# Farama-Foundation/Miniworld

Hardware: NVIDIA H100
Metric: env steps/sec (higher is better)
Workload: dtype f64+f32

## Files before the change

### miniworld_b200/csrc/mwb.cu

```cuda
#include <math.h>
#include <stdio.h>
#include <stdlib.h>
#include <string.h>

#include <algorithm>
#include <string>
#include <vector>

#include "../../include/mwb.h"
#include "raster.cuh"
#include "visibility.cuh"
#include "reset.cuh"

#ifndef MWB_HOSTSIM
#include <cuda_runtime.h>
#endif

#define MWB_MAX_ENTS_CAP 32
#define MWB_STAGE_QUAD_BYTES_HOST 16384

static thread_local std::string g_err;
static int fail(int code, const std::string& msg) {
  g_err = msg;
  return code;
}

#ifdef MWB_HOSTSIM
typedef void* stream_t;
static int dev_alloc(void** p, size_t n) {
  *p = calloc(1, n ? n : 1);
  return *p ? 0 : -1;
}
static void dev_free(void* p) { free(p); }
static int h2d(void* d, const void* h, size_t n, stream_t) { memcpy(d, h, n); return 0; }
static int d2h(void* h, const void* d, size_t n, stream_t) { memcpy(h, d, n); return 0; }
static int dev_memset(void* d, int v, size_t n) { memset(d, v, n); return 0; }
static int sync_stream(stream_t) { return 0; }
static bool is_device_ptr(const void*) { return false; }
#else
typedef cudaStream_t stream_t;
#define CK(call)                                                                              \
  do {                                                                                        \
    cudaError_t e_ = (call);                                                                  \
    if (e_ != cudaSuccess)                                                                    \
      return fail(MWB_ECUDA, std::string(#call) + " (mwb.cu:" + std::to_string(__LINE__) + "): " + cudaGetErrorString(e_)); \
  } while (0)
static int dev_alloc(void** p, size_t n) { return cudaMalloc(p, n ? n : 1) == cudaSuccess ? 0 : -1; }
static void dev_free(void* p) { cudaFree(p); }
static int h2d(void* d, const void* h, size_t n, stream_t s) {
  return cudaMemcpyAsync(d, h, n, cudaMemcpyHostToDevice, s) == cudaSuccess ? 0 : -1;
}
static int d2h(void* h, const void* d, size_t n, stream_t s) {
  return cudaMemcpyAsync(h, d, n, cudaMemcpyDeviceToHost, s) == cudaSuccess ? 0 : -1;
}
static int dev_memset(void* d, int v, size_t n) {
  return cudaMemset(d, v, n) == cudaSuccess && cudaStreamSynchronize(cudaStreamLegacy) == cudaSuccess ? 0 : -1;
}
static int sync_stream(stream_t s) { return cudaStreamSynchronize(s) == cudaSuccess ? 0 : -1; }
static bool is_device_ptr(const void* p) {
  if (!p) return false;
  cudaPointerAttributes a;
  if (cudaPointerGetAttributes(&a, p) != cudaSuccess) {
    cudaGetLastError();
    return false;
  }
  return a.type == cudaMemoryTypeDevice || a.type == cudaMemoryTypeManaged;
}
#endif

struct WorldUpload {
  int32_t env, num_slots, agent_slot, carrying, step_count, num_picked, hold, pad1;
  double cam[4];
  double envp[12];
  mwb_entity ents[MWB_MAX_ENTS_CAP];
  mwb_rng_state rng;
};

#define MWB_D2H_CHUNKS 16

struct mwb_handle {
  mwb_config cfg;
  DevState S;
  RenderAssets A;
  std::vector<void*> allocs;
  stream_t stream;
  int64_t launches;
  int32_t* d_actions;
  double* d_step_params;
  double* d_reward;
  uint8_t* d_term;
  uint8_t* d_trunc;
  uint8_t* d_obs;
  int obs_format;
  size_t obs_px_bytes;
  size_t d_obs_bytes;
  float* d_depth;
  int32_t* d_ids;
  int* d_overflow;
  WorldUpload* d_upload;
  int tri_cap;
  bool smem_tris;
  int stage_bytes;
  bool have_params, have_protos, have_template;
  bool have_level_table;
  std::vector<LevelDev> levels;
  std::vector<int32_t> env_level;
  std::vector<mwb_op> ops_h;
  int geom_blocks;
  bool profiling;
  bool frames_copied;
  int obs_peer_hint;
  const void* peer_checked;
  bool peer_result;
  bool obs_is_peer;
  int k2_static_smem;
  TriRec* vis_tris;
  ViewSpec view;
  int k2_parts;
#ifndef MWB_HOSTSIM
  cudaStream_t copy_stream;
  cudaEvent_t chunk_done[MWB_D2H_CHUNKS], copies_done;
#endif
#ifndef MWB_HOSTSIM
  std::vector<cudaEvent_t> ev_k1, ev_k2;
  cudaEvent_t last_done;
  cudaStream_t last_stream;
  bool last_valid;
#endif
#ifndef MWB_HOSTSIM
  struct AtlasEntry* atlas;
#endif
  std::vector<int> mesh_counts;
  void* mesh_tris_buf;
  void* mesh_bbox_buf;
  void* mesh_bin_idx_buf;
  void* mesh_bin_off_buf;
  void *tex_desc, *texels, *mesh_desc, *mesh_pos, *mesh_nrm, *mesh_uv, *mesh_rgb, *mesh_tex, *protos, *ops, *maze, *maze_cdf;
};

#ifndef MWB_HOSTSIM
struct AtlasEntry {
  int device;
  uint64_t hash;
  size_t texels;
  int refs;
  cudaArray_t arr;
  cudaTextureObject_t obj;
  float iw, ih;
  std::vector<float> ax, ay;
};
static std::vector<AtlasEntry*> g_atlases;
static void release_texture_objects(mwb_handle* h) {
  AtlasEntry* e = h->atlas;
  h->atlas = nullptr;
  if (!e || --e->refs > 0) return;
  for (size_t k = 0; k < g_atlases.size(); ++k)
    if (g_atlases[k] == e) g_atlases.erase(g_atlases.begin() + k);
  cudaDestroyTextureObject(e->obj);
  cudaFreeArray(e->arr);
  delete e;
}
#endif

template <typename T>
static int alloc_arr(mwb_handle* h, T** p, size_t count) {
  void* q = nullptr;
  if (dev_alloc(&q, count * sizeof(T)) != 0) return fail(MWB_ECUDA, "device allocation failed");
  dev_memset(q, 0, count * sizeof(T));
  h->allocs.push_back(q);
  *p = (T*)q;
  return 0;
}

#ifndef MWB_HOSTSIM
static int stream_enter(mwb_handle* h, stream_t s) {
  if (h->last_valid && h->last_stream != s) CK(cudaStreamWaitEvent(s, h->last_done, 0));
  return 0;
}
static int stream_leave(mwb_handle* h, stream_t s) {
  CK(cudaEventRecord(h->last_done, s));
  h->last_stream = s;
  h->last_valid = true;
  return 0;
}
#else
// ... 363 lines not shown
  h->tex_desc = h->texels = h->mesh_desc = h->mesh_pos = h->mesh_nrm = h->mesh_uv = h->mesh_rgb = h->mesh_tex = nullptr;
  h->protos = h->ops = h->maze = h->maze_cdf = nullptr;
  h->mesh_tris_buf = nullptr;
  h->mesh_bbox_buf = nullptr;
  h->mesh_bin_idx_buf = h->mesh_bin_off_buf = nullptr;
  memset(&h->view, 0, sizeof(ViewSpec));
  h->vis_tris = nullptr;
  h->obs_format = MWB_OBS_HWC_U8;
  h->obs_px_bytes = 3;
  h->obs_peer_hint = -1;
  h->peer_checked = nullptr;
  h->peer_result = h->obs_is_peer = false;
  h->k2_static_smem = 19456;
  memset(&h->S, 0, sizeof(DevState));
  memset(&h->A, 0, sizeof(RenderAssets));
#ifndef MWB_HOSTSIM
  if (cudaStreamCreateWithFlags(&h->stream, cudaStreamNonBlocking) != cudaSuccess ||
      cudaStreamCreateWithFlags(&h->copy_stream, cudaStreamNonBlocking) != cudaSuccess) {
    delete h;
    return fail(MWB_ECUDA, "cudaStreamCreate failed");
  }
  for (int c = 0; c < MWB_D2H_CHUNKS; ++c) cudaEventCreateWithFlags(&h->chunk_done[c], cudaEventDisableTiming);
  cudaEventCreateWithFlags(&h->copies_done, cudaEventDisableTiming);
  cudaEventCreateWithFlags(&h->last_done, cudaEventDisableTiming);
  h->last_stream = h->stream;
  h->last_valid = false;
#else
  h->stream = nullptr;
#endif
  DevState& S = h->S;
  const size_t N = cfg->num_envs, E = cfg->max_ents;
  S.N = cfg->num_envs;
  S.E = cfg->max_ents;
  S.R = cfg->max_rooms;
  S.Q = (cfg->max_quads + 1) & ~1;
  S.S = cfg->max_segs;
  S.shared_geom = cfg->shared_geometry;
  S.obs_w = cfg->obs_width;
  S.obs_h = cfg->obs_height;
  S.msaa = cfg->msaa_samples;
  S.domain_rand = cfg->domain_rand;
  S.autoreset = cfg->autoreset;
  {
    LevelDev L0;
    memset(&L0, 0, sizeof(L0));
    L0.rule_kind = cfg->rule_kind;
    L0.rule_arg = cfg->rule_arg;
    L0.max_episode_steps = cfg->max_episode_steps;
    h->levels.assign(1, L0);
    h->env_level.assign(N, 0);
    S.num_levels = 1;
  }
  const size_t G = cfg->shared_geometry ? 1 : N;
  h->geom_blocks = (int)G;
  int rc = 0;
#define AL(field, count) if (!rc) rc = alloc_arr(h, &S.field, (count))
  AL(ent_proto, E * N); AL(ent_px, E * N); AL(ent_py, E * N); AL(ent_pz, E * N); AL(ent_dir, E * N);
  AL(ent_col, E * 3 * N); AL(ent_size, E * N); AL(num_slots, N); AL(agent_slot, N); AL(carrying, N); AL(step_count, N);
  AL(num_picked, N); AL(needs_reset, N); AL(episodes_done, 1); AL(cam, 4 * N); AL(envp, 12 * N); AL(ghost_slot, N);
  AL(ghost_proto, N); AL(ghost_pose, 4 * N); AL(ghost_col, 3 * N);
  AL(rng_s_hi, N); AL(rng_s_lo, N); AL(rng_inc_hi, N); AL(rng_inc_lo, N); AL(rng_has32, N); AL(rng_cache, N);
  AL(num_rooms, G); AL(num_quads, G); AL(num_segs, G);
  AL(rooms, G * S.R); AL(quads, G * S.Q + 2); AL(segs, G * S.S); AL(room_tex, N * S.R * 3);
  AL(mesh_seg, N * E); AL(cam_trig, 6 * N); AL(ent_cs, E * 2 * N);
#undef AL
  LevelDev* d_levels = nullptr;
  int32_t* d_env_level = nullptr;
  if (!rc) rc = alloc_arr(h, &d_levels, MWB_LEVEL_CAP);
  if (!rc) rc = alloc_arr(h, &d_env_level, N);
  S.levels = d_levels;
  S.env_level = d_env_level;
  if (!rc) rc = alloc_arr(h, &h->d_actions, N);
  if (!rc) rc = alloc_arr(h, &h->d_step_params, 3 * N);
  if (!rc) rc = alloc_arr(h, &h->d_reward, N);
  if (!rc) rc = alloc_arr(h, &h->d_term, N);
  if (!rc) rc = alloc_arr(h, &h->d_trunc, N);
  if (!rc) rc = alloc_arr(h, &h->d_obs, N * (size_t)S.obs_w * S.obs_h * 3);
  h->d_obs_bytes = N * (size_t)S.obs_w * S.obs_h * 3;
  if (!rc) rc = alloc_arr(h, &h->d_depth, N * (size_t)S.obs_w * S.obs_h);
  if (!rc) rc = alloc_arr(h, &h->d_ids, N);
  if (!rc) rc = alloc_arr(h, &h->d_overflow, 1);
  S.fault = h->d_overflow;
  if (!rc) rc = alloc_arr(h, &h->d_upload, N);
  if (rc) {
    mwb_destroy(h);
    return rc;
  }
#ifndef MWB_HOSTSIM
  {
    float* lut = nullptr;
    if (alloc_arr(h, &lut, 65536)) {
      mwb_destroy(h);
      return fail(MWB_ECUDA, "depth table allocation failed");
    }
    depth_lut_kernel<<<256, 256, 0, h->stream>>>(lut);
    h->launches++;
    S.depth_lut = lut;
  }
#endif
  dev_memset(S.ent_proto, 0xFF, E * N * sizeof(int32_t));
  dev_memset(S.ghost_slot, 0xFF, N * sizeof(int32_t));
  dev_memset(S.carrying, 0xFF, N * sizeof(int32_t));
  {
    int sms = 132;
#ifndef MWB_HOSTSIM
    if (cudaDeviceGetAttribute(&sms, cudaDevAttrMultiProcessorCount, cfg->device) != cudaSuccess) {
      cudaGetLastError();
      sms = 132;
    }
#endif
    const int slots = 4 * 3 * sms;
    const int halves = ((cfg->obs_width + 7) / 8) * ((cfg->obs_height + 3) / 4);
    const int base = (halves + 149) / 150, want = (slots + cfg->num_envs - 1) / cfg->num_envs;
    const int maxp = halves / 30 > 1 ? halves / 30 : 1;
    h->k2_parts = base > want ? base : want;
    if (h->k2_parts > maxp) h->k2_parts = maxp;
    if (h->k2_parts < 1) h->k2_parts = 1;
  }
  h->tri_cap = 2 * (cfg->max_quads + 6 * cfg->max_ents) + 2;
  h->smem_tris = h->tri_cap <= 512;
  if (!h->smem_tris) {
    TriRec* buf = nullptr;
    if (alloc_arr(h, &buf, (size_t)N * h->k2_parts * h->tri_cap)) {
      mwb_destroy(h);
      return fail(MWB_ECUDA, "triangle list allocation failed");
    }
    S.room_tris = buf;
  }
  h->stage_bytes = (int)(((size_t)cfg->max_quads * sizeof(mwb_quad) + 15) & ~(size_t)15);
  if (h->stage_bytes > MWB_STAGE_QUAD_BYTES_HOST) h->stage_bytes = 0;
#ifndef MWB_HOSTSIM
  {
    cudaFuncAttributes fa;
    if (cudaFuncGetAttributes(&fa, k2_kernels[k2_index(h)]) == cudaSuccess) {
      h->k2_static_smem = (int)fa.sharedSizeBytes;
    } else {
      cudaGetLastError();
      h->k2_static_smem = 19456;
    }
  }
  const int smem = k2_smem_bytes(h) + 16384;
  if (ensure_k2_smem(h, smem)) {
    mwb_destroy(h);
    return fail(MWB_ECUDA, "cudaFuncSetAttribute(MaxDynamicSharedMemorySize) failed");
  }
  if (getenv("MWB_DEBUG")) {
    int nb = 0;
    const int launch_smem = k2_smem_bytes(h);
    cudaOccupancyMaxActiveBlocksPerMultiprocessor(&nb, k2_kernels[k2_index(h)], k2_threads(h), launch_smem);
    fprintf(stderr, "[mwb] K2 %d threads, %dx MSAA: dynamic smem %d B (local destination), parts %d, resident blocks/SM %d\n",
            k2_threads(h), h->S.msaa, launch_smem, h->k2_parts, nb);
  }
#endif
  *out = h;
  return MWB_OK;
}

extern "C" int mwb_destroy(mwb_handle* h) {
  if (!h) return MWB_OK;
#ifndef MWB_HOSTSIM
  cudaSetDevice(h->cfg.device);
  if (h->last_valid) cudaStreamSynchronize(h->last_stream);
  cudaStreamSynchronize(h->stream);
#endif
  for (void* p : h->allocs) dev_free(p);
  void* extra[] = {h->tex_desc, h->texels, h->mesh_desc, h->mesh_pos, h->mesh_nrm, h->mesh_uv, h->mesh_rgb, h->mesh_tex,
// ... 695 lines not shown
  } else {
    flag_write_kernel<<<1, 1, 0, s>>>(dev_ptr, value);
    CK(cudaGetLastError());
  }
  return MWB_OK;
#else
  return fail(MWB_ENOCUDA, "host simulator has no streams");
#endif
}

extern "C" int mwb_flag_wait_geq(void* stream, const uint32_t* dev_ptr, uint32_t value) {
#ifndef MWB_HOSTSIM
  if (!dev_ptr) return fail(MWB_EINVAL, "null argument");
  flag_init();
  cudaStream_t s = (cudaStream_t)stream;
  if (g_flag_mode == 0) {
    if (g_wait32(s, (unsigned long long)(uintptr_t)dev_ptr, value, 0u ) != 0)
      return fail(MWB_ECUDA, "cuStreamWaitValue32 failed");
  } else {
    flag_wait_kernel<<<1, 1, 0, s>>>(dev_ptr, value);
    CK(cudaGetLastError());
  }
  return MWB_OK;
#else
  return fail(MWB_ENOCUDA, "host simulator has no streams");
#endif
}

extern "C" int mwb_flag_mode(void) {
#ifndef MWB_HOSTSIM
  flag_init();
  return g_flag_mode;
#else
  return -1;
#endif
}

#ifndef MWB_HOSTSIM
static void prof_mark(mwb_handle* h, std::vector<cudaEvent_t>& v, stream_t s) {
  if (!h->profiling) return;
  cudaEvent_t e;
  if (cudaEventCreate(&e) != cudaSuccess) return;
  cudaEventRecord(e, s);
  v.push_back(e);
}
static double prof_drain(std::vector<cudaEvent_t>& v, int64_t* count) {
  double ms = 0.0;
  *count = 0;
  for (size_t k = 0; k + 1 < v.size(); k += 2) {
    float t = 0.0f;
    cudaEventSynchronize(v[k + 1]);
    if (cudaEventElapsedTime(&t, v[k], v[k + 1]) == cudaSuccess) {
      ms += t;
      ++*count;
    }
  }
  for (cudaEvent_t e : v) cudaEventDestroy(e);
  v.clear();
  return ms;
}
#endif

extern "C" int mwb_profile(mwb_handle* h, int enable) {
  if (!h) return fail(MWB_EINVAL, "null handle");
  h->profiling = enable != 0;
  return MWB_OK;
}

extern "C" int mwb_profile_read(mwb_handle* h, double* k1_ms, double* k2_ms, int64_t* k1_launches, int64_t* k2_launches) {
  if (!h) return fail(MWB_EINVAL, "null handle");
  double a = 0.0, b = 0.0;
  int64_t na = 0, nb = 0;
#ifndef MWB_HOSTSIM
  a = prof_drain(h->ev_k1, &na);
  b = prof_drain(h->ev_k2, &nb);
#endif
  if (k1_ms) *k1_ms = a;
  if (k2_ms) *k2_ms = b;
  if (k1_launches) *k1_launches = na;
  if (k2_launches) *k2_launches = nb;
  return MWB_OK;
}

static int launch_k2(mwb_handle* h, uint8_t* obs, float* depth, int env0, int count, stream_t s) {
#ifndef MWB_HOSTSIM
  if (obs != h->peer_checked) {
    cudaPointerAttributes pa;
    h->peer_checked = obs;
    h->peer_result = obs && cudaPointerGetAttributes(&pa, obs) == cudaSuccess && pa.type == cudaMemoryTypeDevice &&
                     pa.device != h->cfg.device;
    cudaGetLastError();
  }
  h->obs_is_peer = h->obs_peer_hint >= 0 ? h->obs_peer_hint != 0 : h->peer_result;
  const int smem = k2_smem_bytes(h), fstage = k2_frame_stage_bytes(h);
  const K2Layout lay = k2_layout(h->smem_tris, h->tri_cap, h->stage_bytes, k2_halves_per_part(h->S.obs_w, h->S.obs_h, h->k2_parts), fstage);
  if (ensure_k2_smem(h, smem)) return fail(MWB_ECUDA, "cudaFuncSetAttribute(MaxDynamicSharedMemorySize) failed");
  prof_mark(h, h->ev_k2, s);
  k2_kernels[k2_index(h)]<<<count * h->k2_parts, k2_threads(h), smem, s>>>(h->S, h->A, h->view, h->obs_format, obs, depth, env0,
                                                                          h->k2_parts, h->tri_cap, h->stage_bytes, fstage, lay,
                                                                          h->d_overflow);
  prof_mark(h, h->ev_k2, s);
  h->launches++;
  CK(cudaGetLastError());
#endif
  return MWB_OK;
}

static int launch_render(mwb_handle* h, uint8_t* obs, float* depth, stream_t s, uint8_t* host_obs = nullptr,
                         float* host_depth = nullptr) {
  if (!h->A.tex) return fail(MWB_ESTATE, "textures not uploaded");
#ifndef MWB_HOSTSIM
  {
    const long long threads = (long long)h->S.N * (6 + 2 * h->S.E);
    frame_trig_kernel<<<(unsigned)((threads + 127) / 128), 128, 0, s>>>(h->S);
    h->launches++;
    CK(cudaGetLastError());
  }
  if (h->S.mesh_cap > 0) {
    mesh_setup_kernel<<<dim3(h->S.N, h->S.E), 256, 0, s>>>(h->S, h->A, h->view);
    h->launches++;
    CK(cudaGetLastError());
  }
  const int N = h->S.N;
  const size_t px = (size_t)h->S.obs_w * h->S.obs_h;
  const bool pipelined = (host_obs || host_depth) && N >= 256;
  int chunks = pipelined ? MWB_D2H_CHUNKS : 1;
  while (chunks > 1 && N / chunks < 256) --chunks;
  for (int c = 0; c < chunks; ++c) {
    const int e0 = (int)((long long)N * c / chunks), e1 = (int)((long long)N * (c + 1) / chunks);
    int rc = launch_k2(h, obs, depth, e0, e1 - e0, s);
    if (rc) return rc;
    if (pipelined) {
      CK(cudaEventRecord(h->chunk_done[c], s));
      CK(cudaStreamWaitEvent(h->copy_stream, h->chunk_done[c], 0));
      if (host_obs)
        CK(cudaMemcpyAsync(host_obs + (size_t)e0 * px * h->obs_px_bytes, obs + (size_t)e0 * px * h->obs_px_bytes,
                           (size_t)(e1 - e0) * px * h->obs_px_bytes,
                           cudaMemcpyDeviceToHost, h->copy_stream));
      if (host_depth)
        CK(cudaMemcpyAsync(host_depth + (size_t)e0 * px, depth + (size_t)e0 * px, (size_t)(e1 - e0) * px * sizeof(float),
                           cudaMemcpyDeviceToHost, h->copy_stream));
    }
  }
  if (pipelined) {
    h->frames_copied = true;
    CK(cudaEventRecord(h->copies_done, h->copy_stream));
    CK(cudaStreamWaitEvent(s, h->copies_done, 0));
  }
#else
  hostsim_render(h->S, h->A, h->view, h->obs_format, obs, depth);
#endif
  return MWB_OK;
}

static int finish_outputs(mwb_handle* h, uint8_t* obs, bool obs_host, float* depth, bool depth_host, double* reward,
                          uint8_t* term, uint8_t* trunc, stream_t s, bool user_stream) {
  const size_t N = h->S.N, px = (size_t)h->S.obs_w * h->S.obs_h;
  int rc = 0;
  bool any_host = false;
  if (obs && obs_host) { if (!h->frames_copied) rc |= d2h(obs, h->d_obs, N * px * h->obs_px_bytes, s); any_host = true; }
  if (depth && depth_host) { if (!h->frames_copied) rc |= d2h(depth, h->d_depth, N * px * sizeof(float), s); any_host = true; }
  h->frames_copied = false;
  if (reward && !is_device_ptr(reward)) { rc |= d2h(reward, h->d_reward, N * sizeof(double), s); any_host = true; }
  if (term && !is_device_ptr(term)) { rc |= d2h(term, h->d_term, N, s); any_host = true; }
  if (trunc && !is_device_ptr(trunc)) { rc |= d2h(trunc, h->d_trunc, N, s); any_host = true; }
  if (rc) return fail(MWB_ECUDA, "readback failed");
  if (stream_leave(h, s)) return MWB_ECUDA;
  if (any_host || !user_stream)
    if (sync_stream(s) != 0) return fail(MWB_ECUDA, "stream sync failed");
  return MWB_OK;
}

extern "C" int mwb_step(mwb_handle* h, const int32_t* actions, const double* step_params, uint8_t* obs, float* depth,
                        double* reward, uint8_t* terminated, uint8_t* truncated, void* stream) {
  if (!h || !actions) return fail(MWB_EINVAL, "null argument");
  if (!h->have_params || !h->have_protos) return fail(MWB_ESTATE, "params / protos not set");
  stream_t s = stream ? (stream_t)stream : h->stream;
  if (stream_enter(h, s)) return MWB_ECUDA;
  const size_t N = h->S.N;
  const int32_t* d_act = actions;
  if (!is_device_ptr(actions)) {
    if (h2d(h->d_actions, actions, N * sizeof(int32_t), s) != 0) return fail(MWB_ECUDA, "action upload failed");
    d_act = h->d_actions;
  }
  const double* d_sp = nullptr;
  if (step_params) {
    if (is_device_ptr(step_params)) {
      d_sp = step_params;
    } else {
      if (h2d(h->d_step_params, step_params, 3 * N * sizeof(double), s) != 0) return fail(MWB_ECUDA, "upload failed");
      d_sp = h->d_step_params;
    }
  }
  double* d_rew = reward && is_device_ptr(reward) ? reward : h->d_reward;
  uint8_t* d_te = terminated && is_device_ptr(terminated) ? terminated : h->d_term;
  uint8_t* d_tr = truncated && is_device_ptr(truncated) ? truncated : h->d_trunc;
#ifndef MWB_HOSTSIM
  prof_mark(h, h->ev_k1, s);
  step_kernel<<<(unsigned)((N + 3) / 4), 128, 0, s>>>(h->S, d_act, d_sp, d_rew, d_te, d_tr);
  prof_mark(h, h->ev_k1, s);
  h->launches++;
  CK(cudaGetLastError());
#else
  for (size_t i = 0; i < N; ++i) step_one(h->S, (int)i, d_act, d_sp, d_rew, d_te, d_tr);
#endif
  const bool obs_host = obs && !is_device_ptr(obs), depth_host = depth && !is_device_ptr(depth);
  if (obs || depth) {
    int rc = launch_render(h, obs ? (obs_host ? h->d_obs : obs) : nullptr, depth ? (depth_host ? h->d_depth : depth) : nullptr, s,
                           obs_host ? obs : nullptr, depth_host ? depth : nullptr);
    if (rc) return rc;
  }
  return finish_outputs(h, obs, obs_host, depth, depth_host, reward, terminated, truncated, s, stream != nullptr);
}
// ... 384 lines not shown
```

### miniworld_b200/csrc/raster.cuh

```cuda
#pragma once
#include "raster_core.cuh"

#define MWB_TILE_CAP 16

struct K2Layout {
  int order_off, zkey_off, slot_off, cnt_off, list_off, tmp_off, stage_off, end;
};
static inline
#ifdef __CUDACC__
__host__ __device__
#endif
K2Layout k2_layout(bool smem_tris, int tri_cap, int stage_bytes, int halves_per_part, int frame_stage_bytes) {
  K2Layout L;
  const int tri_bytes = smem_tris ? tri_cap * (int)sizeof(TriRec) : 0;
  const int cap2 = (tri_cap + 1) & ~1;
  L.order_off = tri_bytes;
  L.zkey_off = L.order_off + cap2 * 2;
  L.slot_off = L.zkey_off + tri_cap * 4;
  L.cnt_off = L.slot_off + cap2 * 2;
  L.list_off = L.cnt_off + ((halves_per_part + 1) & ~1) * 2;
  L.tmp_off = L.list_off + halves_per_part * MWB_TILE_CAP * 2;
  const int lists_end = L.tmp_off + halves_per_part * MWB_TILE_CAP * 2, quads_end = tri_bytes + stage_bytes;
  L.stage_off = ((lists_end > quads_end ? lists_end : quads_end) + 15) & ~15;
  L.end = L.stage_off + frame_stage_bytes;
  return L;
}
static inline
#ifdef __CUDACC__
__host__ __device__
#endif
int k2_halves_per_part(int W, int H, int parts) {
  const int tiles_x = (W + 7) >> 3, n_halves = tiles_x * ((H + 3) >> 2);
  int per = (n_halves + parts - 1) / parts;
  if (parts > 1) per = (per + tiles_x - 1) / tiles_x * tiles_x;
  return per;
}

#ifdef __CUDACC__

#define MWB_MAX_SEGS (2 + MWB_MAX_DRAWN)
#define MWB_EQ_CAP 96
#define MWB_SORT_LIMIT 512
#define MWB_STAGE_QUAD_BYTES 16384

__device__ __forceinline__ uint32_t smem_u32(const void* p) { return (uint32_t)__cvta_generic_to_shared(p); }
__device__ __forceinline__ void mbar_init(uint64_t* bar, int count) {
  asm volatile("mbarrier.init.shared::cta.b64 [%0], %1;" ::"r"(smem_u32(bar)), "r"(count));
  asm volatile("fence.mbarrier_init.release.cluster;" ::: "memory");
}
__device__ __forceinline__ void tma_bulk_g2s(void* dst_smem, const void* src_gmem, uint32_t bytes, uint64_t* bar) {
  asm volatile("mbarrier.arrive.expect_tx.shared::cta.b64 _, [%0], %1;" ::"r"(smem_u32(bar)), "r"(bytes) : "memory");
  asm volatile("cp.async.bulk.shared::cluster.global.mbarrier::complete_tx::bytes [%0], [%1], %2, [%3];" ::"r"(
                   smem_u32(dst_smem)),
               "l"(src_gmem), "r"(bytes), "r"(smem_u32(bar))
               : "memory");
}
__device__ __forceinline__ void mbar_wait(uint64_t* bar, uint32_t parity) {
  uint32_t done = 0;
  while (!done) {
    asm volatile(
        "{\n\t.reg .pred p;\n\tmbarrier.try_wait.parity.shared::cta.b64 p, [%1], %2;\n\tselp.u32 %0, 1, 0, p;\n\t}"
        : "=r"(done)
        : "r"(smem_u32(bar)), "r"(parity)
        : "memory");
  }
}

__global__ void frame_trig_kernel(DevState S) {
  const int per = 6 + 2 * S.E;
  const long long g = (long long)blockIdx.x * blockDim.x + threadIdx.x;
  if (g >= (long long)S.N * per) return;
  const int k = (int)(g / S.N), i = (int)(g % S.N);
  const size_t N = S.N;
  if (k < 6) {
    double ang[3];
    camera_angles(S, i, ang);
    S.cam_trig[(size_t)k * N + i] = (k & 1) ? mwb_libm::sin_glibc(ang[k >> 1]) : mwb_libm::cos_glibc(ang[k >> 1]);
    return;
  }
  const int e = (k - 6) >> 1, j = (k - 6) & 1;
  const int p = e == S.ghost_slot[i] ? S.ghost_proto[i] : (e < S.num_slots[i] ? S.ent_proto[e * N + i] : -1);
  if (p < 0) return;
  const double dir = entity_pose(S, i, e).dir;
  const double deg = S.protos[p].deg_form ? d_div(d_mul(dir, 180.0), 3.141592653589793) : d_mul(dir, 57.29577951308232);
  const double rad = d_div(d_mul((double)(float)deg, 3.141592653589793), 180.0);
  S.ent_cs[((size_t)e * 2 + j) * N + i] = (float)(j ? mwb_libm::sin_glibc(rad) : mwb_libm::cos_glibc(rad));
}

__global__ void __launch_bounds__(256) mesh_setup_kernel(DevState S, RenderAssets A, ViewSpec view) {
  const int i = blockIdx.x, e = blockIdx.y;
  const size_t N = S.N;
  __shared__ Camera cam;
  __shared__ int warp_tot[8];
  __shared__ int box[4];
  const int tid = threadIdx.x, lane = tid & 31, warp = tid >> 5;
  MeshSegInfo* info = S.mesh_seg + (size_t)i * S.E + e;
  const int p = e == S.ghost_slot[i] ? S.ghost_proto[i] : (e < S.num_slots[i] ? S.ent_proto[e * N + i] : -1);
  if (p < 0 || S.protos[p].kind != MWB_KIND_MESH) {
    if (tid == 0) info->count = 0;
    return;
  }
  if (tid == 0) {
    if (view.mode == 1) {
      cam = make_top_camera(S, i, view);
    } else {
      double trig[6];
      for (int k = 0; k < 6; ++k) trig[k] = S.cam_trig[(size_t)k * N + i];
      cam = make_camera(S, i, trig);
    }
    box[0] = box[1] = 0x7fffffff;
    box[2] = box[3] = -1;
  }
  __syncthreads();
  const mwb_proto& pr = S.protos[p];
  const EntPose P = entity_pose(S, i, e);
  const float c = S.ent_cs[((size_t)e * 2 + 0) * N + i], s = S.ent_cs[((size_t)e * 2 + 1) * N + i];
  const int ntris = A.meshes[pr.mesh_id].count;
  TriRec* out = S.mesh_tris + ((size_t)i * S.E + e) * S.mesh_cap;
  uint2* out_bbox = S.mesh_bbox + ((size_t)i * S.E + e) * S.mesh_cap;
  int total = 0;
  int x0 = 0x7fffffff, y0 = 0x7fffffff, x1 = -1, y1 = -1;
  for (int start = 0; start < ntris; start += 256) {
    const int t = start + tid;
    TriRec rec;
    int keep = 0;
    if (t < ntris) {
      TriInput in;
      mesh_triangle(A, pr, P, c, s, t, in);
      keep = finish_triangle(cam, in, S.obs_w, S.obs_h, rec) ? 1 : 0;
    }
    int incl = keep;
#pragma unroll
    for (int d = 1; d < 32; d <<= 1) {
      int v = __shfl_up_sync(0xffffffffu, incl, d);
      if (lane >= d) incl += v;
    }
    if (lane == 31) warp_tot[warp] = incl;
    __syncthreads();
    int woff = 0, chunk = 0;
#pragma unroll
    for (int w = 0; w < 8; ++w) {
      int v = warp_tot[w];
      if (w < warp) woff += v;
      chunk += v;
    }
    if (keep) {
      const int pos = total + woff + incl - 1;
      if (pos < S.mesh_cap) {
        out[pos] = rec;
        out_bbox[pos] = make_uint2((unsigned)rec.bx, (unsigned)rec.by);
      }
      x0 = min(x0, rec.bx & 0xFFFF); x1 = max(x1, rec.bx >> 16);
      y0 = min(y0, rec.by & 0xFFFF); y1 = max(y1, rec.by >> 16);
    }
    total += chunk;
    __syncthreads();
  }
  if (x1 >= 0) {
    atomicMin(&box[0], x0); atomicMin(&box[1], y0);
    atomicMax(&box[2], x1); atomicMax(&box[3], y1);
  }
  __syncthreads();
  const int count = total < S.mesh_cap ? total : S.mesh_cap;
  __shared__ int bin_cnt[MWB_MAX_BINS + 1];
  __shared__ int scan_tot[8];
  int binned = 0;
  const int c0 = box[0] >> 3, c1 = box[2] >> 3, r0 = box[1] >> 2, r1 = box[3] >> 2;
  const int cols = c1 - c0 + 1, rows = r1 - r0 + 1, nbins = box[2] >= 0 ? cols * rows : 0;
  int* off = S.mesh_bin_off + ((size_t)i * S.E + e) * (MWB_MAX_BINS + 1);
  uint16_t* bidx = S.mesh_bin_idx + ((size_t)i * S.E + e) * ((size_t)MWB_BIN_REFS * S.mesh_cap);
  if (nbins > 0 && nbins <= MWB_MAX_BINS && count > 64 && count <= 65535) {
    for (int b = tid; b <= nbins; b += 256) bin_cnt[b] = 0;
    __syncthreads();
    for (int pass = 0; pass < 2; ++pass) {
      for (int t = tid; t < count; t += 256) {
        const uint2 bb = out_bbox[t];
        const int tc0 = max((int)(bb.x & 0xFFFF) >> 3, c0), tc1 = min((int)(bb.x >> 16) >> 3, c1);
        const int tr0 = max((int)(bb.y & 0xFFFF) >> 2, r0), tr1 = min((int)(bb.y >> 16) >> 2, r1);
        const TriRec& T = out[t];
        float A[3], B[3], K[3];
#pragma unroll
        for (int k = 0; k < 3; ++k) { A[k] = T.A[k]; B[k] = T.B[k]; K[k] = T.K[k]; }
        for (int r = tr0; r <= tr1; ++r)
          for (int c = tc0; c <= tc1; ++c) {
            const float fx0 = (float)(c << 3), fy0 = (float)(r << 2);
            if (A[0] * fx0 + B[0] * fy0 + K[0] < 0.0f || A[1] * fx0 + B[1] * fy0 + K[1] < 0.0f ||
                A[2] * fx0 + B[2] * fy0 + K[2] < 0.0f)
              continue;
            const int b = (r - r0) * cols + (c - c0);
            const int pos = atomicAdd(&bin_cnt[b], 1);
            if (pass == 1) bidx[pos] = (uint16_t)t;
          }
      }
      __syncthreads();
      if (pass == 0) {
        const int per = (nbins + 255) / 256, b0 = tid * per;
        int sum = 0;
        for (int k = 0; k < per; ++k)
          if (b0 + k < nbins) sum += bin_cnt[b0 + k];
        int incl = sum;
#pragma unroll
        for (int d = 1; d < 32; d <<= 1) {
          int v = __shfl_up_sync(0xffffffffu, incl, d);
          if (lane >= d) incl += v;
        }
        if (lane == 31) scan_tot[warp] = incl;
        __syncthreads();
        int base = incl - sum;
        for (int w = 0; w < warp; ++w) base += scan_tot[w];
        int refs = 0;
        for (int w = 0; w < 8; ++w) refs += scan_tot[w];
        __syncthreads();
        for (int k = 0; k < per; ++k)
          if (b0 + k < nbins) {
            const int cnt = bin_cnt[b0 + k];
            bin_cnt[b0 + k] = base;
            off[b0 + k] = base;
            base += cnt;
          }
        if (tid == 0) off[nbins] = refs;
        binned = refs <= MWB_BIN_REFS * S.mesh_cap ? 1 : 0;
        __syncthreads();
        if (!binned) break;
      }
    }
  }
  if (tid == 0) {
    info->count = count;
    info->bx = box[2] >= 0 ? (box[0] | (box[2] << 16)) : 0;
    info->by = box[3] >= 0 ? (box[1] | (box[3] << 16)) : 0;
    info->binned = binned;
  }
}

__global__ void depth_lut_kernel(float* __restrict__ lut) {
  const uint32_t c = blockIdx.x * blockDim.x + threadIdx.x;
  if (c < 65536u) lut[c] = depth_code_to_metres(c);
}

template <int MSAA, int THREADS, int MINB>
__global__ void __launch_bounds__(THREADS, MINB)
render_kernel(DevState S, RenderAssets A, ViewSpec view, int fmt, uint8_t* __restrict__ obs, float* __restrict__ depth, int env0,
              int parts, int tri_cap, int stage_bytes, int frame_stage_bytes, K2Layout lay, int* __restrict__ overflow) {
  constexpr int WARPS = THREADS / 32;
  extern __shared__ __align__(16) unsigned char smem_raw[];
  const int i = env0 + (int)blockIdx.x / parts, part = (int)blockIdx.x % parts;
  const size_t tri_bytes = S.room_tris ? 0 : (size_t)tri_cap * sizeof(TriRec);
  TriRec* tris = S.room_tris ? S.room_tris + ((size_t)i * parts + part) * tri_cap : reinterpret_cast<TriRec*>(smem_raw);
  __shared__ Camera cam;
  __shared__ FrameMap fmap;
  __shared__ Segment segs[MWB_MAX_SEGS];
  __shared__ int seg_count[MWB_MAX_SEGS];
  __shared__ int warp_tot[WARPS];
  __shared__ __align__(8) uint64_t quad_bar;
  struct __align__(16) WarpScratch {
    uint32_t keys[MSAA][32];
    uint32_t items[MWB_EQ_CAP];
    int chunk[32];
    uint8_t stage[4][24];
  };
  __shared__ WarpScratch wscratch[WARPS];

  const int tid = threadIdx.x, lane = tid & 31, warp = tid >> 5;
  const int W = S.obs_w, H = S.obs_h;

  const mwb_quad* gquads = env_quads(S, i);
  const int nq = S.num_quads[geom_index(S, i)];
  const uint32_t quad_bytes = ((uint32_t)nq * (uint32_t)sizeof(mwb_quad) + 15u) & ~15u;
  const bool staged = quad_bytes > 0 && quad_bytes <= (uint32_t)stage_bytes;
  mwb_quad* squads = reinterpret_cast<mwb_quad*>(smem_raw + tri_bytes);
  uint16_t* order = reinterpret_cast<uint16_t*>(smem_raw + lay.order_off);
  float* zkey = reinterpret_cast<float*>(smem_raw + lay.zkey_off);
  uint16_t* tri_slot = reinterpret_cast<uint16_t*>(smem_raw + lay.slot_off);
  uint16_t* tile_cnt = reinterpret_cast<uint16_t*>(smem_raw + lay.cnt_off);
  uint16_t* tile_list = reinterpret_cast<uint16_t*>(smem_raw + lay.list_off);
  uint16_t* tile_tmp = reinterpret_cast<uint16_t*>(smem_raw + lay.tmp_off);
  uint8_t* fstage = smem_raw + lay.stage_off;
  __shared__ float ent_cs[MWB_MAX_DRAWN][2];
  __shared__ int next_half;
  if (tid == 0) mbar_init(&quad_bar, 1);
  if (tid < MWB_MAX_SEGS) seg_count[tid] = 0;
  __syncthreads();
  if (tid == 0 && staged) tma_bulk_g2s(squads, gquads, quad_bytes, &quad_bar);
  if (tid == 0) {
    if (view.mode == 1) {
      cam = make_top_camera(S, i, view);
    } else {
      double tr[6];
#pragma unroll
      for (int k = 0; k < 6; ++k) tr[k] = S.cam_trig[(size_t)k * S.N + i];
      cam = make_camera(S, i, tr);
    }
  } else if (tid == 32) {
    fmap = build_frame_map(S, i, view.mode == 1 && view.render_agent != 0);
  } else if (tid >= 64 && tid < 64 + 2 * MWB_MAX_DRAWN) {
    const int e = (tid - 64) >> 1;
    if (e < S.num_slots[i] && e < S.E) ent_cs[e][tid & 1] = S.ent_cs[((size_t)e * 2 + (tid & 1)) * S.N + i];
  }
  __syncthreads();
  if (staged) mbar_wait(&quad_bar, 0);
  const mwb_quad* quads = staged ? squads : gquads;

  const int tiles_x = (W + 7) >> 3;
  const float inv_tiles_x = 1.0f / (float)tiles_x;
  const int halves_y = (H + 3) >> 2;
  const int n_halves = tiles_x * halves_y, per_part = k2_halves_per_part(W, H, parts);
  const int h_begin = min(n_halves, part * per_part), h_end = min(n_halves, h_begin + per_part);
  const int band_row0 = (h_begin / tiles_x) << 2;

  int ntris = 0;
  for (int start = 0; start < fmap.n_tasks; start += THREADS) {
    const int task = start + tid;
    TriRec rec;
    int keep = 0, seg = 0;
    if (task < fmap.n_tasks) keep = task_triangle(S, A, cam, fmap, quads, i, task, W, H, rec, seg, ent_cs) ? 1 : 0;
    const int keep_other = __shfl_xor_sync(0xffffffffu, keep, 1);
    const int seg_other = __shfl_xor_sync(0xffffffffu, seg, 1);
    if (!keep && keep_other) {
      empty_record(rec);
      seg = seg_other;
      keep = 1;
    }
    int incl = keep;
#pragma unroll
    for (int d = 1; d < 32; d <<= 1) {
      int v = __shfl_up_sync(0xffffffffu, incl, d);
      if (lane >= d) incl += v;
    }
    if (lane == 31) warp_tot[warp] = incl;
    __syncthreads();
    int woff = 0, total = 0;
#pragma unroll
    for (int w = 0; w < WARPS; ++w) {
      int v = warp_tot[w];
      if (w < warp) woff += v;
      total += v;
    }
    if (keep) {
      const int pos = ntris + woff + incl - 1;
      if (pos < tri_cap) {
        tris[pos] = rec;
        atomicAdd(&seg_count[seg], 1);
      }
    }
    ntris += total;
    __syncthreads();
  }
  const int n_res = ntris < tri_cap ? ntris : tri_cap;
  for (int t = tid; t < n_res; t += THREADS) {
    const TriRec& T = tris[t];
    const float x0 = (float)(T.bx & 0xFFFF), x1 = (float)((T.bx >> 16) + 1), y0 = (float)(T.by & 0xFFFF), y1 = (float)((T.by >> 16) + 1);
    zkey[t] = T.Zc + fminf(T.Za * x0, T.Za * x1) + fminf(T.Zb * y0, T.Zb * y1);
  }
  if (tid == 0) {
    next_half = h_begin + WARPS;
    if (ntris > tri_cap) atomicAdd(overflow, 1);
    int smem_pos = 0, slot = 0;
    const int last = fmap.n_ents + (fmap.agent_task >= 0 ? 1 : 0);
    for (int k = 0; k <= last; ++k) {
      Segment& sg = segs[k];
      if (k == 0 || k > fmap.n_ents || fmap.ent_kind[k - 1] == MWB_KIND_BOX) {
        sg.tris = tris + smem_pos;
        sg.bbox = nullptr;
        sg.bin_idx = nullptr;
        sg.bin_off = nullptr;
        sg.count = seg_count[k];
        smem_pos += sg.count;
        sg.bx = (W - 1) << 16;
        sg.by = (H - 1) << 16;
      } else {
        const int e = fmap.ent_slot[k - 1];
        const MeshSegInfo mi = S.mesh_seg[(size_t)i * S.E + e];
        sg.tris = S.mesh_tris + ((size_t)i * S.E + e) * S.mesh_cap;
        sg.bbox = S.mesh_bbox + ((size_t)i * S.E + e) * S.mesh_cap;
        sg.bin_idx = mi.binned ? S.mesh_bin_idx + ((size_t)i * S.E + e) * ((size_t)MWB_BIN_REFS * S.mesh_cap) : nullptr;
        sg.bin_off = mi.binned ? S.mesh_bin_off + ((size_t)i * S.E + e) * (MWB_MAX_BINS + 1) : nullptr;
        sg.count = mi.count;
        sg.bx = mi.bx;
        sg.by = mi.by;
      }
      sg.base = slot;
      slot += (sg.count + 1) & ~1;
    }
// ... 317 lines not shown
```

Baseline: 4.153 million.

## Precompute per-env camera and frame map in a separate kernel, TMA-load into render

Moves per-environment camera construction and frame-map building out of the render kernel into a new lightweight frame_view_kernel that writes one FrameView per environment. The render kernel then pulls the FrameView into shared memory with a bulk TMA copy on the same mbarrier as the quad staging. This stops the serial single-thread setup from being repeated in every block for every part, at the cost of an extra launch and a global round trip. The start profiling mark moves before the new kernel.

Measured after the change: 4.173 million, median of 6. About the same (+0.5%).

```diff
diff --git a/miniworld_b200/csrc/mwb.cu b/miniworld_b200/csrc/mwb.cu
--- a/miniworld_b200/csrc/mwb.cu
+++ b/miniworld_b200/csrc/mwb.cu
@@ -101,6 +101,9 @@
   int tri_cap;
   bool smem_tris;
   int stage_bytes;
+#ifndef MWB_HOSTSIM
+  FrameView* frame_views;
+#endif
   bool have_params, have_protos, have_template;
   bool have_level_table;
   std::vector<LevelDev> levels;
@@ -630,6 +633,9 @@
   if (!rc) rc = alloc_arr(h, &h->d_overflow, 1);
   S.fault = h->d_overflow;
   if (!rc) rc = alloc_arr(h, &h->d_upload, N);
+#ifndef MWB_HOSTSIM
+  if (!rc) rc = alloc_arr(h, &h->frame_views, N);
+#endif
   if (rc) {
     mwb_destroy(h);
     return rc;
@@ -1491,7 +1497,7 @@
   return MWB_OK;
 }
 
-static int launch_k2(mwb_handle* h, uint8_t* obs, float* depth, int env0, int count, stream_t s) {
+static int launch_k2(mwb_handle* h, uint8_t* obs, float* depth, int env0, int count, stream_t s, bool mark_start) {
 #ifndef MWB_HOSTSIM
   if (obs != h->peer_checked) {
     cudaPointerAttributes pa;
@@ -1504,8 +1510,8 @@
   const int smem = k2_smem_bytes(h), fstage = k2_frame_stage_bytes(h);
   const K2Layout lay = k2_layout(h->smem_tris, h->tri_cap, h->stage_bytes, k2_halves_per_part(h->S.obs_w, h->S.obs_h, h->k2_parts), fstage);
   if (ensure_k2_smem(h, smem)) return fail(MWB_ECUDA, "cudaFuncSetAttribute(MaxDynamicSharedMemorySize) failed");
-  prof_mark(h, h->ev_k2, s);
-  k2_kernels[k2_index(h)]<<<count * h->k2_parts, k2_threads(h), smem, s>>>(h->S, h->A, h->view, h->obs_format, obs, depth, env0,
+  if (mark_start) prof_mark(h, h->ev_k2, s);
+  k2_kernels[k2_index(h)]<<<count * h->k2_parts, k2_threads(h), smem, s>>>(h->S, h->A, h->frame_views, h->obs_format, obs, depth, env0,
                                                                           h->k2_parts, h->tri_cap, h->stage_bytes, fstage, lay,
                                                                           h->d_overflow);
   prof_mark(h, h->ev_k2, s);
@@ -1531,13 +1537,17 @@
     CK(cudaGetLastError());
   }
   const int N = h->S.N;
+  prof_mark(h, h->ev_k2, s);
+  frame_view_kernel<<<(unsigned)((2LL * N + 127) / 128), 128, 0, s>>>(h->S, h->view, h->frame_views);
+  h->launches++;
+  CK(cudaGetLastError());
   const size_t px = (size_t)h->S.obs_w * h->S.obs_h;
   const bool pipelined = (host_obs || host_depth) && N >= 256;
   int chunks = pipelined ? MWB_D2H_CHUNKS : 1;
   while (chunks > 1 && N / chunks < 256) --chunks;
   for (int c = 0; c < chunks; ++c) {
     const int e0 = (int)((long long)N * c / chunks), e1 = (int)((long long)N * (c + 1) / chunks);
-    int rc = launch_k2(h, obs, depth, e0, e1 - e0, s);
+    int rc = launch_k2(h, obs, depth, e0, e1 - e0, s, c > 0);
     if (rc) return rc;
     if (pipelined) {
       CK(cudaEventRecord(h->chunk_done[c], s));
diff --git a/miniworld_b200/csrc/raster.cuh b/miniworld_b200/csrc/raster.cuh
--- a/miniworld_b200/csrc/raster.cuh
+++ b/miniworld_b200/csrc/raster.cuh
@@ -48,8 +48,10 @@
   asm volatile("mbarrier.init.shared::cta.b64 [%0], %1;" ::"r"(smem_u32(bar)), "r"(count));
   asm volatile("fence.mbarrier_init.release.cluster;" ::: "memory");
 }
+__device__ __forceinline__ void mbar_arrive_expect_tx(uint64_t* bar, uint32_t bytes) {
+  asm volatile("mbarrier.arrive.expect_tx.shared::cta.b64 _, [%0], %1;" ::"r"(smem_u32(bar)), "r"(bytes) : "memory");
+}
 __device__ __forceinline__ void tma_bulk_g2s(void* dst_smem, const void* src_gmem, uint32_t bytes, uint64_t* bar) {
-  asm volatile("mbarrier.arrive.expect_tx.shared::cta.b64 _, [%0], %1;" ::"r"(smem_u32(bar)), "r"(bytes) : "memory");
   asm volatile("cp.async.bulk.shared::cluster.global.mbarrier::complete_tx::bytes [%0], [%1], %2, [%3];" ::"r"(
                    smem_u32(dst_smem)),
                "l"(src_gmem), "r"(bytes), "r"(smem_u32(bar))
@@ -85,6 +87,28 @@
   const double deg = S.protos[p].deg_form ? d_div(d_mul(dir, 180.0), 3.141592653589793) : d_mul(dir, 57.29577951308232);
   const double rad = d_div(d_mul((double)(float)deg, 3.141592653589793), 180.0);
   S.ent_cs[((size_t)e * 2 + j) * N + i] = (float)(j ? mwb_libm::sin_glibc(rad) : mwb_libm::cos_glibc(rad));
+}
+
+struct __align__(16) FrameView {
+  Camera cam;
+  FrameMap fmap;
+};
+__global__ void frame_view_kernel(DevState S, ViewSpec view, FrameView* __restrict__ out) {
+  const long long g = (long long)blockIdx.x * blockDim.x + threadIdx.x;
+  if (g >= 2LL * S.N) return;
+  const int k = (int)(g / S.N), i = (int)(g % S.N);
+  if (k == 0) {
+    if (view.mode == 1) {
+      out[i].cam = make_top_camera(S, i, view);
+    } else {
+      double tr[6];
+#pragma unroll
+      for (int q = 0; q < 6; ++q) tr[q] = S.cam_trig[(size_t)q * S.N + i];
+      out[i].cam = make_camera(S, i, tr);
+    }
+  } else {
+    out[i].fmap = build_frame_map(S, i, view.mode == 1 && view.render_agent != 0);
+  }
 }
 
 __global__ void __launch_bounds__(256) mesh_setup_kernel(DevState S, RenderAssets A, ViewSpec view) {
@@ -240,15 +264,15 @@
 
 template <int MSAA, int THREADS, int MINB>
 __global__ void __launch_bounds__(THREADS, MINB)
-render_kernel(DevState S, RenderAssets A, ViewSpec view, int fmt, uint8_t* __restrict__ obs, float* __restrict__ depth, int env0,
-              int parts, int tri_cap, int stage_bytes, int frame_stage_bytes, K2Layout lay, int* __restrict__ overflow) {
+render_kernel(DevState S, RenderAssets A, const FrameView* __restrict__ views, int fmt, uint8_t* __restrict__ obs,
+              float* __restrict__ depth, int env0, int parts, int tri_cap, int stage_bytes, int frame_stage_bytes, K2Layout lay,
+              int* __restrict__ overflow) {
   constexpr int WARPS = THREADS / 32;
   extern __shared__ __align__(16) unsigned char smem_raw[];
   const int i = env0 + (int)blockIdx.x / parts, part = (int)blockIdx.x % parts;
   const size_t tri_bytes = S.room_tris ? 0 : (size_t)tri_cap * sizeof(TriRec);
   TriRec* tris = S.room_tris ? S.room_tris + ((size_t)i * parts + part) * tri_cap : reinterpret_cast<TriRec*>(smem_raw);
-  __shared__ Camera cam;
-  __shared__ FrameMap fmap;
+  __shared__ FrameView fview;
   __shared__ Segment segs[MWB_MAX_SEGS];
   __shared__ int seg_count[MWB_MAX_SEGS];
   __shared__ int warp_tot[WARPS];
@@ -281,24 +305,18 @@
   if (tid == 0) mbar_init(&quad_bar, 1);
   if (tid < MWB_MAX_SEGS) seg_count[tid] = 0;
   __syncthreads();
-  if (tid == 0 && staged) tma_bulk_g2s(squads, gquads, quad_bytes, &quad_bar);
   if (tid == 0) {
-    if (view.mode == 1) {
-      cam = make_top_camera(S, i, view);
-    } else {
-      double tr[6];
-#pragma unroll
-      for (int k = 0; k < 6; ++k) tr[k] = S.cam_trig[(size_t)k * S.N + i];
-      cam = make_camera(S, i, tr);
-    }
-  } else if (tid == 32) {
-    fmap = build_frame_map(S, i, view.mode == 1 && view.render_agent != 0);
+    mbar_arrive_expect_tx(&quad_bar, (uint32_t)sizeof(FrameView) + (staged ? quad_bytes : 0u));
+    tma_bulk_g2s(&fview, views + i, (uint32_t)sizeof(FrameView), &quad_bar);
+    if (staged) tma_bulk_g2s(squads, gquads, quad_bytes, &quad_bar);
   } else if (tid >= 64 && tid < 64 + 2 * MWB_MAX_DRAWN) {
     const int e = (tid - 64) >> 1;
     if (e < S.num_slots[i] && e < S.E) ent_cs[e][tid & 1] = S.ent_cs[((size_t)e * 2 + (tid & 1)) * S.N + i];
   }
   __syncthreads();
-  if (staged) mbar_wait(&quad_bar, 0);
+  mbar_wait(&quad_bar, 0);
+  const Camera& cam = fview.cam;
+  const FrameMap& fmap = fview.fmap;
   const mwb_quad* quads = staged ? squads : gquads;
 
   const int tiles_x = (W + 7) >> 3;
```
